# deadskull7/One-Stop-for-COVID-19-Infection-and-Lung-Segmentation-plus-Classification

Measured on AMD Instinct MI355X. Metric: CT images/sec (fwd+bwd) U-Net 512x512x1 bs16, higher is better.
Workload: dtype f32 storage / accumulate / parameters; conv products as a two-term fp16 split (3 fp16 MFMAs per multiply, ~2^-22 per product; --algo 2 = strict fp32); 1 GPU; U-Net infection seg (task1 graph T1:853-916), 512x512x1, batch 16/GPU, fp32, fwd+loss+bwd+Keras-Adam; BASELINE.json configs[1]; storage=fp32, global_batch=16, parallelism=dp1, deterministic=False, bn_fold=2

## Files before the change

### include/unet_hip.h

```cpp
#ifndef UNET_HIP_H
#define UNET_HIP_H
#include <stddef.h>
#include <stdint.h>

#ifdef __cplusplus
extern "C" {
#endif

#define UNET_ABI_VERSION 16

typedef struct unet_ctx unet_ctx;
typedef struct unet_model unet_model;
typedef uint16_t unet_bf16;
enum { UNET_DTYPE_F32 = 0, UNET_DTYPE_BF16 = 1 };

enum { UNET_OK = 0, UNET_E_ARG = -1, UNET_E_HIP = -2, UNET_E_SHAPE = -3, UNET_E_STATE = -4, UNET_E_NODEV = -5 };

enum { UNET_ALGO_AUTO = 0, UNET_ALGO_NAIVE = 1, UNET_ALGO_MFMA = 2 };

int32_t unet_abi_version(void);
int32_t unet_ctx_create(int32_t device_id, unet_ctx** out);
void unet_ctx_destroy(unet_ctx* ctx);
const char* unet_last_error(const unet_ctx* ctx);
int32_t unet_ctx_set_profiling(unet_ctx* ctx, int32_t on);
enum { UNET_OPT_RELU_BITS = 1, UNET_OPT_BN_FOLD = 2, UNET_OPT_ENC_BN_FUSED = 3, UNET_OPT_BN_CONCAT_ANALYTIC = 4, UNET_OPT_BN_FUSE_STATS = 5, UNET_OPT_DETERMINISTIC = 6,
       UNET_OPT_HEAD_FUSED = 7, UNET_OPT_SKIP_RAW = 8, UNET_OPT_POOL_SUMS_FUSED = 9, UNET_OPT_HEAD_BWD_FUSED = 10, UNET_OPT_CONV_PP = 13 };
int32_t unet_ctx_set_option(unet_ctx* ctx, int32_t option, int32_t value);
int32_t unet_ctx_get_option(unet_ctx* ctx, int32_t option);

enum { UNET_ACT_NONE = 0, UNET_ACT_RELU = 1, UNET_ACT_ELU = 2 };
enum { UNET_MASK_NONE = 0, UNET_MASK_RELU = 1, UNET_MASK_ELU = 2, UNET_MASK_ELU_DROP = 3, UNET_MASK_RELU_BITS = 9  };

size_t unet_conv3x3_w_ws_floats(int32_t cin, int32_t cout);
int32_t unet_conv3x3_pick_algo(int32_t algo, int32_t wd, int32_t cin, int32_t cout);
double unet_conv3x3_exec_ratio(int32_t algo, int32_t h, int32_t wd, int32_t cin, int32_t cout);
double unet_conv3x3_wgrad_exec_ratio(int32_t algo, int32_t h, int32_t wd, int32_t cin, int32_t cout);
int32_t unet_request_bn_stats(unet_ctx*, int32_t c);
int32_t unet_relu_bits_supported(int32_t algo, int32_t h, int32_t wd, int32_t cin, int32_t cout);
size_t unet_relu_bits_bytes(int32_t n, int32_t h, int32_t wd, int32_t c);
int32_t unet_request_relu_bits(unet_ctx*, void* bits);
int32_t unet_allow_k_slices(unet_ctx*);
// ... 16 lines not shown
int32_t unet_conv3x3_bwd_weights(unet_ctx*, const float* x, const float* dy, float* dw, float* db,
                                 void* ws, size_t ws_bytes, int32_t n, int32_t h, int32_t wd,
                                 int32_t cin, int32_t cout, int32_t algo, void* stream);

int32_t unet_convT2x2_fwd(unet_ctx*, const float* x, const float* w, const float* bias, float* y,
                          int32_t ldy, int32_t n, int32_t h, int32_t wd, int32_t cin, int32_t cout,
                          int32_t algo, void* stream);
int32_t unet_convT2x2_bwd_data(unet_ctx*, const float* dy, int32_t lddy, const float* w,
                               const float* relu_src, float* dx, int32_t n, int32_t h, int32_t wd,
                               int32_t cin, int32_t cout, int32_t algo, void* stream);
size_t unet_convT2x2_bwd_weights_ws_bytes(int32_t n, int32_t h, int32_t wd, int32_t cin, int32_t cout);
int32_t unet_convT2x2_bwd_weights(unet_ctx*, const float* x, const float* dy, int32_t lddy,
                                  float* dw, float* db, void* ws, size_t ws_bytes, int32_t n,
                                  int32_t h, int32_t wd, int32_t cin, int32_t cout, int32_t algo,
                                  void* stream);

int32_t unet_bn_stats(unet_ctx*, const float* x, int32_t ldx, double* sums, int64_t pixels,
                      int32_t c, void* stream);
int32_t unet_bn_stats_concat(unet_ctx*, const float* x_up, int32_t ldx, const double* src_sums, double src_count, const float* src_gamma,
                             const float* src_beta, double* sums, int64_t pixels, int32_t c_up, int32_t c_skip, void* stream);
int32_t unet_bn_finalize_train(unet_ctx*, const double* sums, double count, const float* gamma,
                               const float* beta, float* moving_mean, float* moving_var,
                               float* bnp, int32_t c, void* stream);
int32_t unet_bn_finalize_infer(unet_ctx*, const float* gamma, const float* beta,
                               const float* moving_mean, const float* moving_var, float* bnp,
                               int32_t c, void* stream);
int32_t unet_bn_apply(unet_ctx*, const float* x, int32_t ldx, const float* bnp, float* y,
                      int32_t ldy, int64_t pixels, int32_t c, void* stream);
int32_t unet_bn_bwd_stats(unet_ctx*, const float* dy, int32_t lddy, const float* x, int32_t ldx,
                          const float* bnp, double* sums, int64_t pixels, int32_t c, void* stream);
// ... 248 lines not shown
```

### one-stop-for-covid-19-infection-and-lung-segmentation-plus-classification_amd/_lib.py

```python
from __future__ import annotations

import ctypes as C
import os

_HERE = os.path.dirname(os.path.abspath(__file__))
LIB_PATH = os.environ.get("COVIDSEG_AMD_LIB") or os.path.join(_HERE, "libunet_hip.so")
ABI_VERSION = 16
COMM_HANDLE_BYTES, COMM_MAX_WORLD, COMM_MAX_DOUBLES = 64, 8, 2048

ALGO_AUTO, ALGO_NAIVE, ALGO_MFMA = 0, 1, 2
OPTIONS = {"relu_bits": 1, "bn_fold": 2, "enc_bn_fused": 3, "bn_concat_analytic": 4, "bn_fuse_stats": 5, "deterministic": 6, "head_fused": 7, "skip_raw": 8, "pool_sums_fused": 9, "head_bwd_fused": 10, "conv_pp": 13}
ARCH_UNET, ARCH_UNETPP, ARCH_CLASSIFIER = 0, 1, 2
LOSSES = {"bce_dice_loss": 0, "binary_crossentropy": 1, "dice_loss": 2, "tversky_loss": 3, "weighted_bce_dice_loss": 4}
DTYPE_F32, DTYPE_BF16 = 0, 1
ACT_NONE, ACT_RELU, ACT_ELU = 0, 1, 2
MASK_NONE, MASK_RELU, MASK_ELU, MASK_ELU_DROP = 0, 1, 2, 3
PROG_FWD_TRAIN, PROG_BWD, PROG_FWD_INFER = 0, 1, 2
SYNC_BN_FWD, SYNC_LOSS, SYNC_BN_BWD, SYNC_GRAD_BUCKET = 0, 1, 2, 3

f32p = C.POINTER(C.c_float)
f64p = C.POINTER(C.c_double)
vp = C.c_void_p
i32, i64, u64, f32, f64, sz = C.c_int32, C.c_int64, C.c_uint64, C.c_float, C.c_double, C.c_size_t


class SyncPoint(C.Structure):
# ... 14 lines not shown
    "unet_conv3x3_wgrad_exec_ratio": (f64, [i32, i32, i32, i32, i32]),
    "unet_request_bn_stats": (i32, [vp, i32]),
    "unet_relu_bits_supported": (i32, [i32, i32, i32, i32, i32]),
    "unet_relu_bits_bytes": (sz, [i32, i32, i32, i32]),
    "unet_request_relu_bits": (i32, [vp, vp]),
    "unet_allow_k_slices": (i32, [vp]),
    "unet_ctx_max_kernel_scratch_bytes": (i32, [vp]),
    "unet_conv3x3_fwd": (i32, [vp, vp, vp, vp, vp, i32, i32, i32, i32, i32, i32, f32, u64, i32, vp, vp]),
    "unet_conv3x3_bwd_data": (i32, [vp, vp, vp, vp, i32, f32, u64, vp, vp, i32, i32, i32, i32, i32, i32, vp]),
    "unet_conv3x3_bwd_weights_ws_bytes": (sz, [i32, i32, i32, i32, i32]),
    "unet_conv3x3_bwd_weights": (i32, [vp, vp, vp, vp, vp, vp, sz, i32, i32, i32, i32, i32, i32, vp]),
    "unet_convT2x2_fwd": (i32, [vp, vp, vp, vp, vp, i32, i32, i32, i32, i32, i32, i32, vp]),
    "unet_convT2x2_bwd_data": (i32, [vp, vp, i32, vp, vp, vp, i32, i32, i32, i32, i32, i32, vp]),
    "unet_convT2x2_bwd_weights_ws_bytes": (sz, [i32, i32, i32, i32, i32]),
    "unet_convT2x2_bwd_weights": (i32, [vp, vp, vp, i32, vp, vp, vp, sz, i32, i32, i32, i32, i32, i32, vp]),
    "unet_cast_f32_to_bf16": (i32, [vp, vp, vp, i64, vp]),
    "unet_cast_bf16_to_f32": (i32, [vp, vp, vp, i64, vp]),
    "unet_conv3x3_fwd_bf16": (i32, [vp, vp, vp, vp, vp, i32, i32, i32, i32, i32, i32, f32, u64, vp, vp]),
    "unet_conv3x3_first_fwd_bf16": (i32, [vp, vp, vp, vp, vp, i32, i32, i32, i32, i32, f32, u64, vp]),
    "unet_conv3x3_bwd_data_bf16": (i32, [vp, vp, vp, vp, i32, f32, u64, vp, vp, i32, i32, i32, i32, i32, vp]),
    "unet_conv3x3_bwd_weights_ws_bytes_bf16": (sz, [i32, i32, i32, i32, i32]),
    "unet_conv3x3_bwd_weights_bf16": (i32, [vp, vp, vp, vp, vp, vp, sz, i32, i32, i32, i32, i32, vp]),
    "unet_conv3x3_first_bwd_weights_bf16": (i32, [vp, vp, vp, vp, vp, vp, sz, i32, i32, i32, i32, vp]),
    "unet_convT2x2_fwd_bf16": (i32, [vp, vp, vp, vp, vp, i32, i32, i32, i32, i32, i32, vp, vp]),
    "unet_convT2x2_bwd_data_bf16": (i32, [vp, vp, i32, vp, vp, vp, i32, i32, i32, i32, i32, vp, vp]),
    "unet_convT2x2_bwd_weights_ws_bytes_bf16": (sz, [i32, i32, i32, i32, i32]),
    "unet_convT2x2_bwd_weights_bf16": (i32, [vp, vp, vp, i32, vp, vp, vp, sz, i32, i32, i32, i32, i32, vp]),
    "unet_bn_stats": (i32, [vp, vp, i32, vp, i64, i32, vp]),
    "unet_bn_stats_bf16": (i32, [vp, vp, i32, vp, i64, i32, vp]),
    "unet_conv3x3_bnfold_supported": (i32, [i32, i32, i32, i32, i32]),
# ... 198 lines not shown
```

### one-stop-for-covid-19-infection-and-lung-segmentation-plus-classification_amd/csrc/common.h

```cpp
#pragma once
#include <hip/hip_runtime.h>
#include <stdint.h>
#include <stdio.h>
#include <set>
#include <string>

#include "../../include/unet_hip.h"

constexpr int UNET_BN_SLOTS = 64, UNET_BN_SLOTS_DET = 1024, UNET_BN_SLOT_DOUBLES = 2048;
struct unet_loss_sel { int32_t kind = UNET_LOSS_BCE_DICE; float alpha = 0.5f, beta = 0.5f; };
inline bool unet_loss_sel_ok(const unet_loss_sel& ls, const float* wm = nullptr, bool need_map = true) {
  if (ls.kind < UNET_LOSS_BCE_DICE || ls.kind > UNET_LOSS_WEIGHTED_BCE_DICE) return false;
  if (ls.kind == UNET_LOSS_TVERSKY && !(ls.alpha > 0.0f && ls.beta > 0.0f && ls.alpha < 1e30f && ls.beta < 1e30f)) return false;
  return !need_map || (ls.kind == UNET_LOSS_WEIGHTED_BCE_DICE) == (wm != nullptr);
}
constexpr int UNET_HEAD_SUMS = 100;
struct unet_ctx {
  int device = 0;
  int num_cu = 256;
  int profiling = 0;
  int opt_relu_bits = 1;
  int opt_bn_fold = 2;
  int opt_enc_bn_fused = 1;
  int opt_bn_concat_analytic = 1;
  int opt_bn_fuse_stats = 1;
  int opt_pool_sums_fused = 1;
  int opt_skip_raw = 1;
  int opt_head_fused = 1;
  int opt_head_bwd_fused = 1;
  int opt_conv_pp = 1;
  int opt_deterministic = 0;
  double* bn_slots = nullptr;
  int bn_nslots() const { return opt_deterministic ? UNET_BN_SLOTS_DET : UNET_BN_SLOTS; }
  void* convt_img = nullptr;
  size_t convt_img_bytes = 0;
  int k_slices_ok = 0;
  void* splitk_ws = nullptr;
  size_t splitk_ws_bytes = 0;
  int stats_req_c = 0;
  const void* stats_in_slots = nullptr;
  int stats_in_slots_c = 0;
  bool stats_in_slots_xs = false;
  unsigned long long* signs_req = nullptr;
  const void* signs_done = nullptr;
  std::set<const void*> big_lds_kernels;
// ... 270 lines not shown
int32_t k_convT_naive_dgrad(unet_ctx*, const float* dy, int lddy, const float* w, const float* mask, float* dx,
                            int n, int h, int wd, int cin, int cout, hipStream_t s);
int32_t k_convT_naive_wgrad(unet_ctx*, const float* x, const float* dy, int lddy, float* dw, float* db, int n,
                            int h, int wd, int cin, int cout, hipStream_t s);
bool mfma_conv3x3_supported(int cin, int cout);
int32_t k_conv3x3_mfma_fwd(unet_ctx*, const float* x, const float* w, const float* bias, const float* mask, int mask_mode,
                           float* y, int n, int h, int wd, int cin, int cout, int act, float rate, uint64_t seed, hipStream_t s);
bool mfma_wgrad_supported(int ca, int cb);
bool mfma_convT_supported(int cin, int cout);
int32_t k_convT_mfma_fwd(unet_ctx*, const float* x, const float* w, const float* bias, float* y, int ldy, int n, int h, int wd,
                         int cin, int cout, hipStream_t s);
int32_t k_convT_mfma_dgrad(unet_ctx*, const float* dy, int lddy, const float* w, const float* mask, float* dx, int n, int h, int wd,
                           int cin, int cout, hipStream_t s);
size_t mfma_convT_wgrad_ws_bytes(int n, int h, int wd, int cin, int cout);
bool h2_convT_wgrad_selected(int algo, int cin, int cout);
size_t h2_convT_wgrad_ws_bytes(int n, int h, int wd, int cin, int cout);
int32_t k_convT_h2_wgrad(unet_ctx*, const float* x, const float* dy, int lddy, float* dw, float* db, void* ws, size_t ws_bytes, int n, int h, int wd, int cin, int cout,
                         hipStream_t s);
int32_t k_convT_mfma_wgrad(unet_ctx*, const float* x, const float* dy, int lddy, float* dw, float* db, void* ws, size_t ws_bytes, int n,
                           int h, int wd, int cin, int cout, hipStream_t s);
size_t mfma_wgrad_ws_bytes(int n, int h, int wd, int cin, int cout);
int32_t k_conv3x3_mfma_wgrad(unet_ctx*, const float* x, const float* dy, float* dw, float* db, void* ws,
                             size_t ws_bytes, int n, int h, int wd, int cin, int cout, hipStream_t s);
bool bf16_conv3x3_supported(int cin, int cout);
bool bf16_convT_supported(int cin, int cout);
bool bf16_wgrad_supported(int ca, int cb);
int32_t k_conv3x3_bf16_fwd(unet_ctx*, const unet_bf16* x, const float* w, const float* bias, const unet_bf16* mask, int mask_mode, unet_bf16* y, int n, int h,
                           int wd, int cin, int cout, int act, float rate, uint64_t seed, unet_bf16* wimg, int flip, hipStream_t s,
                           const unet_bf16* prepared = nullptr);
struct unet_wimg_prep { const float* w; unet_bf16* img; long long tap_stride, sk, sm, total8; int nb, nchunks, flip, m; };
// ... 19 lines not shown
```

### one-stop-for-covid-19-infection-and-lung-segmentation-plus-classification_amd/csrc/kernels_wgrad_h2.hip

```cpp
#include <stdlib.h>

#include <algorithm>

#include "common.h"

namespace {

typedef _Float16 f16x8 __attribute__((ext_vector_type(8)));
typedef _Float16 f16x2 __attribute__((ext_vector_type(2)));
typedef short s16x4 __attribute__((ext_vector_type(4)));
typedef short s16x8 __attribute__((ext_vector_type(8)));
typedef unet_f32x16 f32x16;

__device__ __forceinline__ void split2(float a, float b, unsigned& h, unsigned& m) {
  const f16x2 hh = __builtin_convertvector((unet_f32x2){a, b}, f16x2);
  const f16x2 mm = __builtin_convertvector((unet_f32x2){a - (float)hh[0], b - (float)hh[1]}, f16x2);
  h = __builtin_bit_cast(unsigned, hh); m = __builtin_bit_cast(unsigned, mm);
}
__device__ __forceinline__ float pow2f(int e) { return __uint_as_float((unsigned)(e + 127) << 23); }

__device__ __forceinline__ f16x8 lds_tr_frag(const char* p0, const char* p1) {
  typedef __attribute__((address_space(3))) s16x4 lds_s16x4;
  const s16x4 a = __builtin_amdgcn_ds_read_tr16_b64_v4i16((lds_s16x4*)(p0));
  const s16x4 b = __builtin_amdgcn_ds_read_tr16_b64_v4i16((lds_s16x4*)(p1));
// ... 518 lines not shown
  const long long pairs = (long long)p.tiles_a * p.tiles_b, per = 4LL * ca * cb;
  const long long units = (long long)n * p.strips;
  long long want = std::max<long long>(1, 512 / pairs);
  want = std::min(want, std::max<long long>(1, (64LL << 20) / per));
  p.units = (int)units; p.upb = (int)std::max<long long>(1, units / want);
  const long long ublocks = (units + p.upb - 1) / p.upb;
  long long cps = std::max<long long>(1, want / ublocks);
  cps = std::min<long long>(cps, std::max<long long>(1, h / 4));
  int rpc = (int)((h + cps - 1) / cps); rpc = (rpc + p.R - 1) / p.R * p.R;
  p.rows_per_chunk = rpc; p.chunks_per_strip = (h + rpc - 1) / rpc;
  p.nsplit = (int)(ublocks * p.chunks_per_strip); p.nslabs = p.nsplit;
  p.floats = (size_t)p.nslabs * (per + ca) + wgrad_reduce_scratch_floats(4, ca, cb, ca, p.nslabs);
  return p;
}

struct WgPlanH2 { int WA, WB, WR, tiles_a, tiles_b, strips, rows_per_chunk, chunks_per_strip, nsplit, nslabs, units, upb; size_t floats; };

constexpr int wgrad_h2_rows() { return 2; }

WgPlanH2 plan_wgrad_h2(int n, int h, int w, int ca, int cb) {
  WgPlanH2 p;
  int R = wgrad_h2_rows();
  p.WA = (ca % 64) == 0 ? 2 : 1; p.WB = (cb % 64) == 0 ? 2 : 1;
  p.WR = 4 / (p.WA * p.WB);
  if (p.WR > R) R = 4;
  p.tiles_a = (ca + 32 * p.WA - 1) / (32 * p.WA); p.tiles_b = (cb + 32 * p.WB - 1) / (32 * p.WB); p.strips = (w + 31) / 32;
  const long long pairs = (long long)p.tiles_a * p.tiles_b, per = 9LL * ca * cb;
  const long long units = (long long)n * p.strips;
  const long long target = R == 4 && p.WA * p.WB > 1 ? 256LL : 512LL;
  long long want = std::max<long long>(1, target / pairs);
// ... 99 lines not shown
  const WgPlanT p = plan_wgradT_h2(n, h, wd, cout, cin);
  if (!ws || ws_bytes < p.floats * sizeof(float)) UNET_FAIL(ctx, UNET_E_ARG, "convT wgrad h2: workspace %zu < %zu bytes", ws_bytes, p.floats * sizeof(float));
  float* part = static_cast<float*>(ws);
  const long long S = 4LL * cout * cin + cout;
  const int npairs = p.tiles_a * p.tiles_b;
  const dim3 grid((unsigned)(8 * ((p.nsplit + 7) / 8) * npairs));
  if (p.WA == 2 && p.BW == 2) hipLaunchKernelGGL((wgradT_h2_kernel<2, 2, 1, 1, 2>), grid, dim3(256), 0, s, dy, lddy, x, part, n, h, wd, cout, cin, p.tiles_b, p.strips, p.rows_per_chunk, p.chunks_per_strip,
                                    p.nsplit, npairs, S, p.units, p.upb);
  else if (p.WA == 2) hipLaunchKernelGGL((wgradT_h2_kernel<2, 2, 1, 1>), grid, dim3(256), 0, s, dy, lddy, x, part, n, h, wd, cout, cin, p.tiles_b, p.strips, p.rows_per_chunk, p.chunks_per_strip,
                                    p.nsplit, npairs, S, p.units, p.upb);
  else hipLaunchKernelGGL((wgradT_h2_kernel<1, 2, 2, 2>), grid, dim3(256), 0, s, dy, lddy, x, part, n, h, wd, cout, cin, p.tiles_b, p.strips, p.rows_per_chunk, p.chunks_per_strip, p.nsplit,
                          npairs, S, p.units, p.upb);
  UNET_CHECK_LAUNCH(ctx, "wgradT_h2");
  return k_wgrad_reduce(ctx, part, p.nslabs, 4, cout, cin, cout, dw, db, s);
}
```

### one-stop-for-covid-19-infection-and-lung-segmentation-plus-classification_amd/csrc/model.hip

```cpp
#include <algorithm>
#include <functional>
#include <map>
#include <set>
#include <string>
#include <vector>

#include "common.h"

extern "C" {

int32_t unet_abi_version(void) { return UNET_ABI_VERSION; }

int32_t unet_ctx_create(int32_t device_id, unet_ctx** out) {
  if (!out) return UNET_E_ARG;
  *out = nullptr;
  int ndev = 0;
  if (hipGetDeviceCount(&ndev) != hipSuccess || ndev <= 0 || device_id < 0 || device_id >= ndev) return UNET_E_NODEV;
  hipDeviceProp_t prop;
  if (hipGetDeviceProperties(&prop, device_id) != hipSuccess) return UNET_E_NODEV;
  if (std::string(prop.gcnArchName).rfind("gfx950", 0) != 0) return UNET_E_NODEV;
  unet_ctx* c = new unet_ctx();
  c->device = device_id;
  c->num_cu = prop.multiProcessorCount;
  const size_t sb = sizeof(double) * UNET_BN_SLOTS_DET * UNET_BN_SLOT_DOUBLES;
// ... 20 lines not shown
int32_t unet_ctx_set_profiling(unet_ctx* ctx, int32_t on) { if (!ctx) return UNET_E_ARG; ctx->profiling = on; return UNET_OK; }

static int* ctx_option(unet_ctx* ctx, int32_t option) {
  switch (option) {
    case UNET_OPT_RELU_BITS: return &ctx->opt_relu_bits;
    case UNET_OPT_BN_FOLD: return &ctx->opt_bn_fold;
    case UNET_OPT_ENC_BN_FUSED: return &ctx->opt_enc_bn_fused;
    case UNET_OPT_BN_CONCAT_ANALYTIC: return &ctx->opt_bn_concat_analytic;
    case UNET_OPT_BN_FUSE_STATS: return &ctx->opt_bn_fuse_stats;
    case UNET_OPT_DETERMINISTIC: return &ctx->opt_deterministic;
    case UNET_OPT_HEAD_FUSED: return &ctx->opt_head_fused;
    case UNET_OPT_SKIP_RAW: return &ctx->opt_skip_raw;
    case UNET_OPT_POOL_SUMS_FUSED: return &ctx->opt_pool_sums_fused;
    case UNET_OPT_HEAD_BWD_FUSED: return &ctx->opt_head_bwd_fused;
    case UNET_OPT_CONV_PP: return &ctx->opt_conv_pp;
    default: return nullptr;
  }
}
int32_t unet_ctx_set_option(unet_ctx* ctx, int32_t option, int32_t value) {
  if (!ctx) return UNET_E_ARG;
  int* p = ctx_option(ctx, option);
  const int hi = option == UNET_OPT_BN_FOLD ? 3 : option == UNET_OPT_CONV_PP ? 2 : 1;
  if (!p || value < 0 || value > hi) UNET_FAIL(ctx, UNET_E_ARG, "ctx_set_option: option %d value %d", option, value);
  *p = value;
  return UNET_OK;
}
int32_t unet_ctx_get_option(unet_ctx* ctx, int32_t option) {
  if (!ctx) return UNET_E_ARG;
  const int* p = ctx_option(ctx, option);
  if (!p) UNET_FAIL(ctx, UNET_E_ARG, "ctx_get_option: unknown option %d", option);
// ... 287 lines not shown
}
size_t unet_conv3x3_bwd_weights_ws_bytes_bf16(int32_t n, int32_t h, int32_t wd, int32_t cin, int32_t cout) {
  if (cin == 1) return c1_wgrad_ws_bytes(cout);
  return bf16_wgrad_ws_bytes(n, h, wd, cin, cout);
}
int32_t unet_conv3x3_bwd_weights_bf16(unet_ctx* ctx, const unet_bf16* x, const unet_bf16* dy, float* dw, float* db, void* ws, size_t ws_bytes, int32_t n,
                                      int32_t h, int32_t wd, int32_t cin, int32_t cout, void* stream) {
  if (!ctx || !x || !dy || !dw || !db || n < 1 || h < 1 || wd < 1) UNET_FAIL(ctx, UNET_E_ARG, "conv3x3_bwd_weights_bf16: bad args");
  return k_conv3x3_bf16_wgrad(ctx, x, dy, dw, db, ws, ws_bytes, n, h, wd, cin, cout, as_stream(stream));
}
int32_t unet_conv3x3_first_bwd_weights_bf16(unet_ctx* ctx, const float* x, const unet_bf16* dy, float* dw, float* db, void* ws, size_t ws_bytes, int32_t n,
                                            int32_t h, int32_t wd, int32_t cout, void* stream) {
  if (!ctx || !x || !dy || !dw || !db || n < 1 || h < 1 || wd < 1) UNET_FAIL(ctx, UNET_E_ARG, "conv3x3_first_bwd_weights_bf16: bad args");
  return k_conv3x3_c1_wgrad_bf16(ctx, x, dy, dw, db, ws, ws_bytes, n, h, wd, cout, as_stream(stream));
}
int32_t unet_convT2x2_fwd_bf16(unet_ctx* ctx, const unet_bf16* x, const float* w, const float* bias, unet_bf16* y, int32_t ldy, int32_t n, int32_t h,
                               int32_t wd, int32_t cin, int32_t cout, void* w_ws, void* stream) {
  if (!ctx || !x || !w || !y || !w_ws || ldy < cout || (ldy & 7) || n < 1 || h < 1 || wd < 1) UNET_FAIL(ctx, UNET_E_ARG, "convT_fwd_bf16: bad args");
  return k_convT_bf16_fwd(ctx, x, w, bias, y, ldy, n, h, wd, cin, cout, static_cast<unet_bf16*>(w_ws), as_stream(stream));
}
int32_t unet_convT2x2_bwd_data_bf16(unet_ctx* ctx, const unet_bf16* dy, int32_t lddy, const float* w, const unet_bf16* relu_src, unet_bf16* dx, int32_t n,
                                    int32_t h, int32_t wd, int32_t cin, int32_t cout, void* w_ws, void* stream) {
  if (!ctx || !dy || !w || !dx || !w_ws || lddy < cout || (lddy & 7)) UNET_FAIL(ctx, UNET_E_ARG, "convT_bwd_data_bf16: bad args");
  return k_convT_bf16_dgrad(ctx, dy, lddy, w, relu_src, dx, n, h, wd, cin, cout, static_cast<unet_bf16*>(w_ws), as_stream(stream));
}
size_t unet_convT2x2_bwd_weights_ws_bytes_bf16(int32_t n, int32_t h, int32_t wd, int32_t cin, int32_t cout) { return bf16_convT_wgrad_ws_bytes(n, h, wd, cin, cout); }
int32_t unet_convT2x2_bwd_weights_bf16(unet_ctx* ctx, const unet_bf16* x, const unet_bf16* dy, int32_t lddy, float* dw, float* db, void* ws, size_t ws_bytes,
                                       int32_t n, int32_t h, int32_t wd, int32_t cin, int32_t cout, void* stream) {
  if (!ctx || !x || !dy || !dw || !db || lddy < cout || (lddy & 7)) UNET_FAIL(ctx, UNET_E_ARG, "convT_bwd_weights_bf16: bad args");
  return k_convT_bf16_wgrad(ctx, x, dy, lddy, dw, db, ws, ws_bytes, n, h, wd, cin, cout, as_stream(stream));
// ... 256 lines not shown
    int s = m->H, t = m->W, idx = 0;
    for (auto& l : m->layers) {
      (void)idx;
      if (l.kind != 0) continue;
      int lvl;
      if (l.name == "c5a" || l.name == "c5b") lvl = 4;
      else { int k = l.name[1] - '0'; lvl = (k <= 4) ? k - 1 : 9 - k; }
      int hs = s >> lvl, ts = t >> lvl;
      wgb = std::max(wgb, m->dt ? unet_conv3x3_bwd_weights_ws_bytes_bf16(m->N, hs, ts, l.cin, l.cout) : unet_conv3x3_bwd_weights_ws_bytes(m->N, hs, ts, l.cin, l.cout));
    }
    for (auto& l : m->layers) {
      if (l.kind != 1) continue;
      int k = l.name[1] - '0';
      int lvl = 10 - k;
      wgb = std::max(wgb, m->dt ? bf16_convT_wgrad_ws_bytes(m->N, s >> lvl, t >> lvl, l.cin, l.cout) : unet_convT2x2_bwd_weights_ws_bytes(m->N, s >> lvl, t >> lvl, l.cin, l.cout));
    }
  }
  m->wgrad_ws_bytes = wgb;
  m->off_wgrad_ws = cv.take((wgb + 3) / 4);
  m->ws_floats_train = cv.cur;
}

double nel(const Buf& b) { return (double)b.n * b.h * b.w * b.c; }

#define ADD_OP(vec, nm, fl, by, ...)                          \
  do {                                                        \
    Op _o; _o.name = (nm); _o.flops = (fl); _o.bytes = (by);  \
    _o.run = [=](hipStream_t s) -> int32_t __VA_ARGS__;       \
    (vec).push_back(std::move(_o));                           \
  } while (0)
// ... 408 lines not shown
      const TInfo a = m->tinfo.at(first), b = m->tinfo.at(last_tensor);
      SY.push_back({(int)BW.size() - 1, 3, false, (size_t)a.off * 4, b.off + b.count - a.off});
    };
    bool enc_split = false;
    const int dec[4] = {256, 128, 64, 32};
    for (int k = 9; k >= 6; --k) {
      int c = dec[k - 6]; std::string ks = std::to_string(k);
      std::string prev = (k == 6) ? "c5b" : "c" + std::to_string(k - 1) + "b";
      int cprev = (k == 6) ? 512 : dec[k - 7];
      conv_bwd("c" + ks + "b", "c" + ks + "a", c, c, true, true, "", m->fold_c_off.count("c" + ks + "a") != 0);
      conv_bwd("c" + ks + "a", "bn" + ks, 2 * c, c, true, false, m->fold_off.count("c" + ks + "a") ? "cat" + ks : "");
      flush_def();
      if (!m->fold_c_off.count("c" + ks + "a")) bn_bwd("bn" + ks, "bn" + ks, "cat" + ks, "cat" + ks, 2 * c, 0, m->fold_off.count("c" + ks + "a") != 0);
      const Buf ib = m->act.at(prev), ug = m->grad.at("u" + ks);
      const std::string un = "u" + ks;
      ADD_OP(BW, "convT_wgrad:" + un, 2.0 * 4 * cprev * c * nel(ib) / ib.c, eb * (nel(ib) + nel(ug)), {
        if (dt) return k_convT_bf16_wgrad(ctx, CBF(m->Av(prev)), CBF(m->Dv(un)), ug.ld, m->G(un + "/kernel"), m->G(un + "/bias"), m->wsf(m->off_wgrad_ws), m->wgrad_ws_bytes, ib.n, ib.h,
                                          ib.w, cprev, c, s);
        return unet_convT2x2_bwd_weights(ctx, m->A(prev), m->D(un), ug.ld, m->G(un + "/kernel"), m->G(un + "/bias"), m->wsf(m->off_wgrad_ws), m->wgrad_ws_bytes,
                                         ib.n, ib.h, ib.w, cprev, c, algo, s);
      });
      ADD_OP(BW, "convT_dgrad:" + un, 2.0 * 4 * cprev * c * nel(ib) / ib.c, eb * (2 * nel(ib) + nel(ug)), {
        if (dt) return k_convT_bf16_dgrad(ctx, CBF(m->Dv(un)), ug.ld, m->P(un + "/kernel"), CBF(m->Av(prev)), WBF(m->Dv(prev)), ib.n, ib.h, ib.w, cprev, c, WBF(static_cast<void*>(m->wsf(m->off_wt))), s);
        const auto so = m->sign_off.find(prev);
        const auto pb = m->wprep_b.find(un);
        const void* img = pb == m->wprep_b.end() ? nullptr : m->wsf(pb->second);
        if (so != m->sign_off.end()) return k_convT_h2_dgrad(ctx, m->D(un), ug.ld, m->P(un + "/kernel"), m->wsf(so->second), m->D(prev), ib.n, ib.h, ib.w, cprev, c, s, 1, img);
        if (img) return k_convT_h2_dgrad(ctx, m->D(un), ug.ld, m->P(un + "/kernel"), m->A(prev), m->D(prev), ib.n, ib.h, ib.w, cprev, c, s, 0, img);
        return unet_convT2x2_bwd_data(ctx, m->D(un), ug.ld, m->P(un + "/kernel"), m->A(prev), m->D(prev), ib.n, ib.h, ib.w, cprev, c, algo, s);
      });
      if (k == 7) bucket("u7/kernel", "out/bias");
      if (k == 6) bucket("u6/kernel", "c6b/bias");
    }
    conv_bwd("c5b", "c5a", 512, 512, true, true);
    conv_bwd("c5a", "p4", 256, 512, true, false, "", ctx->opt_enc_bn_fused != 0);
    if (!ctx->opt_enc_bn_fused) bucket("c5a/kernel", "c5b/bias");
    for (int k = 4; k >= 1; --k) {
      int c = ENC[k - 1]; std::string ks = std::to_string(k);
      const Buf xb = m->act.at("bn" + ks), gb = m->grad.at("bn" + ks);
      const std::string bnn = "bn" + ks, pn = "p" + ks;
      const size_t so = m->bn_bsum_off.at(bnn);
      if (ctx->opt_enc_bn_fused) {
        const std::string dn = "bn" + std::to_string(10 - k), cb = "c" + ks + "b";
        const size_t sod = m->bn_bsum_off.at(dn), bod = m->bnp_off.at(dn), bo = m->bnp_off.at(bnn);
        const Buf cbuf = m->act.at(cb), cg = m->grad.at(cb);
// ... 1001 lines not shown
```

Measured before the change: 1065 images/sec.

## Fuse convT 2x2 weight-grad and data-grad into one MFMA kernel for 64->32 layer

```diff
diff --git a/include/unet_hip.h b/include/unet_hip.h
--- a/include/unet_hip.h
+++ b/include/unet_hip.h
@@ -24,7 +24,7 @@
 const char* unet_last_error(const unet_ctx* ctx);
 int32_t unet_ctx_set_profiling(unet_ctx* ctx, int32_t on);
 enum { UNET_OPT_RELU_BITS = 1, UNET_OPT_BN_FOLD = 2, UNET_OPT_ENC_BN_FUSED = 3, UNET_OPT_BN_CONCAT_ANALYTIC = 4, UNET_OPT_BN_FUSE_STATS = 5, UNET_OPT_DETERMINISTIC = 6,
-       UNET_OPT_HEAD_FUSED = 7, UNET_OPT_SKIP_RAW = 8, UNET_OPT_POOL_SUMS_FUSED = 9, UNET_OPT_HEAD_BWD_FUSED = 10, UNET_OPT_CONV_PP = 13 };
+       UNET_OPT_HEAD_FUSED = 7, UNET_OPT_SKIP_RAW = 8, UNET_OPT_POOL_SUMS_FUSED = 9, UNET_OPT_HEAD_BWD_FUSED = 10, UNET_OPT_CONV_PP = 13, UNET_OPT_CONVT_BWD_FUSED = 14 };
 int32_t unet_ctx_set_option(unet_ctx* ctx, int32_t option, int32_t value);
 int32_t unet_ctx_get_option(unet_ctx* ctx, int32_t option);
 
@@ -71,6 +71,11 @@
                                   float* dw, float* db, void* ws, size_t ws_bytes, int32_t n,
                                   int32_t h, int32_t wd, int32_t cin, int32_t cout, int32_t algo,
                                   void* stream);
+int32_t unet_convT2x2_bwd_fused_supported(unet_ctx*, int32_t algo, int32_t cin, int32_t cout);
+size_t unet_convT2x2_bwd_fused_ws_bytes(int32_t n, int32_t h, int32_t wd, int32_t cin, int32_t cout);
+int32_t unet_convT2x2_bwd_fused(unet_ctx*, const float* x, const float* dy, int32_t lddy, const float* w, int32_t relu_mask, float* dx, int32_t accumulate,
+                                float* dw, float* db, void* ws, size_t ws_bytes, int32_t n, int32_t h, int32_t wd, int32_t cin, int32_t cout, int32_t algo,
+                                void* stream);
 
 int32_t unet_bn_stats(unet_ctx*, const float* x, int32_t ldx, double* sums, int64_t pixels,
                       int32_t c, void* stream);
diff --git a/one-stop-for-covid-19-infection-and-lung-segmentation-plus-classification_amd/_lib.py b/one-stop-for-covid-19-infection-and-lung-segmentation-plus-classification_amd/_lib.py
--- a/one-stop-for-covid-19-infection-and-lung-segmentation-plus-classification_amd/_lib.py
+++ b/one-stop-for-covid-19-infection-and-lung-segmentation-plus-classification_amd/_lib.py
@@ -9,7 +9,7 @@
 COMM_HANDLE_BYTES, COMM_MAX_WORLD, COMM_MAX_DOUBLES = 64, 8, 2048
 
 ALGO_AUTO, ALGO_NAIVE, ALGO_MFMA = 0, 1, 2
-OPTIONS = {"relu_bits": 1, "bn_fold": 2, "enc_bn_fused": 3, "bn_concat_analytic": 4, "bn_fuse_stats": 5, "deterministic": 6, "head_fused": 7, "skip_raw": 8, "pool_sums_fused": 9, "head_bwd_fused": 10, "conv_pp": 13}
+OPTIONS = {"relu_bits": 1, "bn_fold": 2, "enc_bn_fused": 3, "bn_concat_analytic": 4, "bn_fuse_stats": 5, "deterministic": 6, "head_fused": 7, "skip_raw": 8, "pool_sums_fused": 9, "head_bwd_fused": 10, "conv_pp": 13, "convt_bwd_fused": 14}
 ARCH_UNET, ARCH_UNETPP, ARCH_CLASSIFIER = 0, 1, 2
 LOSSES = {"bce_dice_loss": 0, "binary_crossentropy": 1, "dice_loss": 2, "tversky_loss": 3, "weighted_bce_dice_loss": 4}
 DTYPE_F32, DTYPE_BF16 = 0, 1
@@ -54,6 +54,9 @@
     "unet_convT2x2_bwd_data": (i32, [vp, vp, i32, vp, vp, vp, i32, i32, i32, i32, i32, i32, vp]),
     "unet_convT2x2_bwd_weights_ws_bytes": (sz, [i32, i32, i32, i32, i32]),
     "unet_convT2x2_bwd_weights": (i32, [vp, vp, vp, i32, vp, vp, vp, sz, i32, i32, i32, i32, i32, i32, vp]),
+    "unet_convT2x2_bwd_fused_supported": (i32, [vp, i32, i32, i32]),
+    "unet_convT2x2_bwd_fused_ws_bytes": (sz, [i32, i32, i32, i32, i32]),
+    "unet_convT2x2_bwd_fused": (i32, [vp, vp, vp, i32, vp, i32, vp, i32, vp, vp, vp, sz, i32, i32, i32, i32, i32, i32, vp]),
     "unet_cast_f32_to_bf16": (i32, [vp, vp, vp, i64, vp]),
     "unet_cast_bf16_to_f32": (i32, [vp, vp, vp, i64, vp]),
     "unet_conv3x3_fwd_bf16": (i32, [vp, vp, vp, vp, vp, i32, i32, i32, i32, i32, i32, f32, u64, vp, vp]),
diff --git a/one-stop-for-covid-19-infection-and-lung-segmentation-plus-classification_amd/csrc/common.h b/one-stop-for-covid-19-infection-and-lung-segmentation-plus-classification_amd/csrc/common.h
--- a/one-stop-for-covid-19-infection-and-lung-segmentation-plus-classification_amd/csrc/common.h
+++ b/one-stop-for-covid-19-infection-and-lung-segmentation-plus-classification_amd/csrc/common.h
@@ -29,6 +29,7 @@
   int opt_head_fused = 1;
   int opt_head_bwd_fused = 1;
   int opt_conv_pp = 1;
+  int opt_convt_bwd_fused = 1;
   int opt_deterministic = 0;
   double* bn_slots = nullptr;
   int bn_nslots() const { return opt_deterministic ? UNET_BN_SLOTS_DET : UNET_BN_SLOTS; }
@@ -329,6 +330,10 @@
                            int cin, int cout, hipStream_t s);
 size_t mfma_convT_wgrad_ws_bytes(int n, int h, int wd, int cin, int cout);
 bool h2_convT_wgrad_selected(int algo, int cin, int cout);
+bool h2_convT_bwd_fused_selected(const unet_ctx* ctx, int algo, int cin, int cout);
+size_t h2_convT_bwd_fused_ws_bytes(int n, int h, int wd, int cin, int cout);
+int32_t k_convT_h2_bwd_fused(unet_ctx*, const float* x, const float* dy, int lddy, const float* w, int relu_mask, float* dx, int accumulate, float* dw, float* db, void* ws,
+                             size_t ws_bytes, int n, int h, int wd, int cin, int cout, hipStream_t s, const void* prepared = nullptr);
 size_t h2_convT_wgrad_ws_bytes(int n, int h, int wd, int cin, int cout);
 int32_t k_convT_h2_wgrad(unet_ctx*, const float* x, const float* dy, int lddy, float* dw, float* db, void* ws, size_t ws_bytes, int n, int h, int wd, int cin, int cout,
                          hipStream_t s);
diff --git a/one-stop-for-covid-19-infection-and-lung-segmentation-plus-classification_amd/csrc/kernels_wgrad_h2.hip b/one-stop-for-covid-19-infection-and-lung-segmentation-plus-classification_amd/csrc/kernels_wgrad_h2.hip
--- a/one-stop-for-covid-19-infection-and-lung-segmentation-plus-classification_amd/csrc/kernels_wgrad_h2.hip
+++ b/one-stop-for-covid-19-infection-and-lung-segmentation-plus-classification_amd/csrc/kernels_wgrad_h2.hip
@@ -556,6 +556,263 @@
   return p;
 }
 
+constexpr int TB_PPL = 32 * 64 + 64, TB_ROWB = 2 * TB_PPL;
+constexpr int TB_A = 2 * TB_ROWB, TB_B = 2 * 32 * 64;
+constexpr int TB_STAGE1 = TB_A + TB_B;
+constexpr int TB_W = 16 * 64 * 32;
+constexpr int TB_PART = 4 * 32 * 128;
+constexpr int TB_SMEM = 2 * TB_STAGE1 + TB_W + TB_PART;
+__device__ __forceinline__ int tb_cell(int p, int c) { return p * 128 + ((c ^ (p & 7)) << 4); }
+
+__global__ __launch_bounds__(256, 2) void convT_bwd_h2_kernel(const float* __restrict__ A, int ldA, const float* __restrict__ B, const unet_bf16* __restrict__ wimg_hdr,
+                                                              float* __restrict__ dX, float* __restrict__ part, int N, int H, int W, int strips, int rows_per_chunk,
+                                                              int chunks_per_strip, int nsplit, long long pstride, int units, int upb, int relu_mask, int accumulate) {
+  constexpr int CA = 32, CB = 64, TAPS = 4;
+  extern __shared__ __attribute__((aligned(16))) char smem[];
+  __shared__ float s_bs[4][64];
+  __shared__ float s_amax[2][4];
+  char* const s_a = smem; char* const s_b = smem + TB_A;
+  char* const s_w = smem + 2 * TB_STAGE1; char* const s_part = s_w + TB_W;
+  const int tid = threadIdx.x, lane = tid & 63, l31 = lane & 31, hi = lane >> 5;
+  const int wave = __builtin_amdgcn_readfirstlane(tid >> 6);
+  const int kp = wave & 1, wb = wave >> 1;
+  const int split = blockIdx.x;
+  if (split >= nsplit) return;
+  const int chunk = split % chunks_per_strip; const int ublk = split / chunks_per_strip;
+  const int ya = chunk * rows_per_chunk;
+  const int yb = ya + rows_per_chunk < H ? ya + rows_per_chunk : H;
+  const int HA = 2 * H, WAI = 2 * W;
+
+  {
+    const uint4* src = reinterpret_cast<const uint4*>(wimg_hdr + 128);
+#pragma unroll
+    for (int k = 0; k < 8; ++k) *reinterpret_cast<uint4*>(s_w + (tid + k * 256) * 16) = src[tid + k * 256];
+  }
+  const float w_unscale = *reinterpret_cast<const float*>(wimg_hdr);
+
+  f32x16 acc[TAPS];
+#pragma unroll
+  for (int t = 0; t < TAPS; ++t)
+#pragma unroll
+    for (int r = 0; r < 16; ++r) acc[t][r] = 0.0f;
+  float bsum = 0.0f;
+  int e_a = 120, e_b = 120;
+
+  const int i16 = lane & 15, g4 = lane >> 4;
+  const int tr_px = kp * 16 + (g4 >> 1) * 8 + (i16 >> 2), tr_ch = ((g4 & 1) * 16 + (i16 & 3) * 4) * 2;
+  const int sw0 = ((g4 >> 1) * 2) & 3;
+  const int a_off0 = tr_px * 64 + ((((tr_ch >> 4) ^ sw0)) << 4) + (tr_ch & 15);
+  const int a_off1 = (tr_px + 4) * 64 + ((((tr_ch >> 4) ^ (sw0 + 1))) << 4) + (tr_ch & 15);
+  const int b_off0 = (wb * 32 + tr_px) * 64 + tr_ch, b_off1 = b_off0 + 4 * 64;
+  const int d_sw = (l31 >> 2) & 3;
+
+  const int q8 = tid & 7, pc = tid >> 3;
+  const int u1 = (ublk + 1) * upb < units ? (ublk + 1) * upb : units;
+  for (int unit = ublk * upb; unit < u1; ++unit) {
+    const int cs = unit % strips, n = unit / strips;
+    const int x0 = cs * 32;
+    const __amdgpu_buffer_rsrc_t rs_a = make_rsrc(A + (long long)n * HA * WAI * ldA, (long long)HA * WAI * ldA * 4);
+    const __amdgpu_buffer_rsrc_t rs_b = make_rsrc(B + (long long)n * H * W * CB, (long long)H * W * CB * 4);
+    int abase_t[2], bbase_t[2], aput[2];
+#pragma unroll
+    for (int half = 0; half < 2; ++half) {
+      const int gx = 2 * x0 + half * 32 + pc;
+      abase_t[half] = gx < WAI ? (gx * ldA + q8 * 4) * 4 : UNET_OOB;
+      const int j = half * 16 + (pc >> 1);
+      aput[half] = (pc & 1) * TB_PPL + j * 64 + ((((q8 >> 1) ^ ((j >> 2) & 3))) << 4) + (q8 & 1) * 8;
+    }
+#pragma unroll
+    for (int sub = 0; sub < 2; ++sub) bbase_t[sub] = x0 + pc < W ? ((x0 + pc) * CB + sub * 32 + q8 * 4) * 4 : UNET_OOB;
+    unet_u32x4 areg[4], breg[2];
+    auto issue_loads = [&](int ys) __attribute__((always_inline)) {
+#pragma unroll
+      for (int row = 0; row < 2; ++row)
+#pragma unroll
+        for (int half = 0; half < 2; ++half) areg[row * 2 + half] = __builtin_amdgcn_raw_buffer_load_b128(rs_a, abase_t[half], (2 * ys + row) * WAI * ldA * 4, 0);
+#pragma unroll
+      for (int sub = 0; sub < 2; ++sub) breg[sub] = __builtin_amdgcn_raw_buffer_load_b128(rs_b, bbase_t[sub], ys * W * CB * 4, 0);
+    };
+    auto post_amax = [&]() __attribute__((always_inline)) {
+      float ma = 0.f, mb = 0.f;
+#pragma unroll
+      for (int k = 0; k < 4; ++k)
+#pragma unroll
+        for (int j = 0; j < 4; ++j) ma = fmaxf(ma, fabsf(__uint_as_float(areg[k][j])));
+#pragma unroll
+      for (int k = 0; k < 2; ++k)
+#pragma unroll
+        for (int j = 0; j < 4; ++j) mb = fmaxf(mb, fabsf(__uint_as_float(breg[k][j])));
+      ma = wave_max_nonneg(ma); mb = wave_max_nonneg(mb);
+      if (lane == 0) { s_amax[0][wave] = ma; s_amax[1][wave] = mb; }
+    };
+    unsigned xsign = 0;
+    float un_x = 0.f;
+    auto store_lds = [&]() __attribute__((always_inline)) {
+      const float ma = fmaxf(fmaxf(s_amax[0][0], s_amax[0][1]), fmaxf(s_amax[0][2], s_amax[0][3]));
+      const float mb = fmaxf(fmaxf(s_amax[1][0], s_amax[1][1]), fmaxf(s_amax[1][2], s_amax[1][3]));
+      const int eba = __builtin_amdgcn_readfirstlane((int)((__float_as_uint(ma) >> 23) & 0xFF));
+      const int ebb = __builtin_amdgcn_readfirstlane((int)((__float_as_uint(mb) >> 23) & 0xFF));
+      int d = 0;
+      if (eba >= 11 && eba - 127 + e_a >= 15) {
+        const int da_ = 138 - eba - e_a;
+        bsum *= pow2f(max(da_, -126));
+        d += da_; e_a = 138 - eba;
+      }
+      if (ebb >= 11 && ebb - 127 + e_b >= 15) { d += 138 - ebb - e_b; e_b = 138 - ebb; }
+      if (d != 0) {
+        const float f = pow2f(max(d, -126));
+#pragma unroll
+        for (int t = 0; t < TAPS; ++t)
+#pragma unroll
+          for (int r = 0; r < 16; ++r) acc[t][r] *= f;
+      }
+      const float sa = pow2f(e_a), sb = pow2f(e_b);
+      un_x = pow2f(max(-e_a, -126)) * w_unscale;
+      auto put = [&](char* dst, const unet_u32x4& v, float sc) __attribute__((always_inline)) {
+        unsigned h0, m0, h1, m1;
+        split2_scaled(__uint_as_float(v[0]), __uint_as_float(v[1]), sc, h0, m0);
+        split2_scaled(__uint_as_float(v[2]), __uint_as_float(v[3]), sc, h1, m1);
+        *reinterpret_cast<uint2*>(dst) = make_uint2(h0, h1);
+        *reinterpret_cast<uint2*>(dst + TB_STAGE1) = make_uint2(m0, m1);
+      };
+#pragma unroll
+      for (int row = 0; row < 2; ++row)
+#pragma unroll
+        for (int half = 0; half < 2; ++half) put(s_a + row * TB_ROWB + aput[half], areg[row * 2 + half], sa);
+      xsign = 0;
+#pragma unroll
+      for (int sub = 0; sub < 2; ++sub) {
+        put(s_b + (sub * 32 + pc) * 64 + q8 * 8, breg[sub], sb);
+#pragma unroll
+        for (int j = 0; j < 4; ++j) xsign |= (__uint_as_float(breg[sub][j]) > 0.f ? 1u : 0u) << (sub * 4 + j);
+      }
+    };
+
+    issue_loads(ya);
+    post_amax();
+    __syncthreads();
+    store_lds();
+    __syncthreads();
+    for (int ys = ya; ys < yb; ++ys) {
+      const bool more = ys + 1 < yb;
+      if (more) issue_loads(ys + 1);
+      {
+        f16x8 ah[4], am[4];
+#pragma unroll
+        for (int ab = 0; ab < 4; ++ab) {
+          const char* ap = s_a + (ab >> 1) * TB_ROWB + (ab & 1) * TB_PPL;
+          ah[ab] = lds_tr_frag(ap + a_off0, ap + a_off1); am[ab] = lds_tr_frag(ap + TB_STAGE1 + a_off0, ap + TB_STAGE1 + a_off1);
+          if (wb == 0) {
+#pragma unroll
+            for (int j = 0; j < 8; ++j) bsum += (float)ah[ab][j] + (float)am[ab][j];
+          }
+        }
+        const f16x8 bh = lds_tr_frag(s_b + b_off0, s_b + b_off1), bm = lds_tr_frag(s_b + TB_STAGE1 + b_off0, s_b + TB_STAGE1 + b_off1);
+#pragma unroll
+        for (int ab = 0; ab < 4; ++ab) acc[ab] = __builtin_amdgcn_mfma_f32_32x32x16_f16(ah[ab], bm, acc[ab], 0, 0, 0);
+#pragma unroll
+        for (int ab = 0; ab < 4; ++ab) acc[ab] = __builtin_amdgcn_mfma_f32_32x32x16_f16(am[ab], bh, acc[ab], 0, 0, 0);
+#pragma unroll
+        for (int ab = 0; ab < 4; ++ab) acc[ab] = __builtin_amdgcn_mfma_f32_32x32x16_f16(ah[ab], bh, acc[ab], 0, 0, 0);
+      }
+      {
+        f32x16 dacc[2];
+#pragma unroll
+        for (int i = 0; i < 2; ++i)
+#pragma unroll
+          for (int r = 0; r < 16; ++r) dacc[i][r] = 0.0f;
+        f16x8 wf[4][2], px[4][2];
+#pragma unroll
+        for (int t = 0; t < 4; ++t)
+#pragma unroll
+          for (int p = 0; p < 2; ++p) {
+            const int kk = kp * 4 + t;
+            wf[t][p] = *reinterpret_cast<const f16x8*>(s_w + ((((kk * 2 + wb) * 2 + p) * 2 + hi) * 512 + l31 * 16));
+            px[t][p] = *reinterpret_cast<const f16x8*>(s_a + p * TB_STAGE1 + kp * TB_ROWB + (t >> 1) * TB_PPL + l31 * 64 + (((((t & 1) * 2 + hi) ^ d_sw)) << 4));
+          }
+#pragma unroll
+        for (int pr = 0; pr < 3; ++pr) {
+          constexpr int PW[3] = {0, 1, 0}, PX[3] = {1, 0, 0};
+#pragma unroll
+          for (int t = 0; t < 4; ++t) dacc[t & 1] = __builtin_amdgcn_mfma_f32_32x32x16_f16(wf[t][PW[pr]], px[t][PX[pr]], dacc[t & 1], 0, 0, 0);
+        }
+        char* const so = s_part + wave * (32 * 128);
+#pragma unroll
+        for (int q = 0; q < 4; ++q)
+          *reinterpret_cast<float4*>(so + tb_cell(l31, hi * 4 + q)) = make_float4(dacc[0][q * 4] + dacc[1][q * 4], dacc[0][q * 4 + 1] + dacc[1][q * 4 + 1],
+                                                                                   dacc[0][q * 4 + 2] + dacc[1][q * 4 + 2], dacc[0][q * 4 + 3] + dacc[1][q * 4 + 3]);
+      }
+      if (more) post_amax();
+      __syncthreads();
+      if (x0 + pc < W) {
+        float* const o = dX + (((long long)n * H + ys) * W + x0 + pc) * CB + q8 * 4;
+#pragma unroll
+        for (int sub = 0; sub < 2; ++sub) {
+          const float4 p0 = *reinterpret_cast<const float4*>(s_part + (sub * 2) * (32 * 128) + tb_cell(pc, q8));
+          const float4 p1 = *reinterpret_cast<const float4*>(s_part + (sub * 2 + 1) * (32 * 128) + tb_cell(pc, q8));
+          float v[4] = {(p0.x + p1.x) * un_x, (p0.y + p1.y) * un_x, (p0.z + p1.z) * un_x, (p0.w + p1.w) * un_x};
+          if (relu_mask) {
+#pragma unroll
+            for (int j = 0; j < 4; ++j) v[j] = ((xsign >> (sub * 4 + j)) & 1u) ? v[j] : 0.f;
+          }
+          float* const q = o + sub * 32;
+          if (accumulate) { const float4 old = *reinterpret_cast<const float4*>(q); v[0] += old.x; v[1] += old.y; v[2] += old.z; v[3] += old.w; }
+          __builtin_nontemporal_store(v[0], q); __builtin_nontemporal_store(v[1], q + 1); __builtin_nontemporal_store(v[2], q + 2); __builtin_nontemporal_store(v[3], q + 3);
+        }
+      }
+      if (more) store_lds();
+      __syncthreads();
+    }
+  }
+  const float un_a = pow2f(max(-e_a, -126));
+  const float un = un_a * pow2f(max(-e_b, -126));
+#pragma unroll
+  for (int t = 0; t < TAPS; ++t)
+#pragma unroll
+    for (int r = 0; r < 16; ++r) acc[t][r] *= un;
+  bsum *= un_a;
+  bsum += __shfl_xor(bsum, 32, 64);
+  float* const img = reinterpret_cast<float*>(smem) + (size_t)wb * (TAPS * 16 * 64);
+  s_bs[wave][lane] = bsum;
+  if (kp == 1) {
+#pragma unroll
+    for (int t = 0; t < TAPS; ++t)
+#pragma unroll
+      for (int r = 0; r < 16; ++r) img[(t * 16 + r) * 64 + lane] = acc[t][r];
+  }
+  __syncthreads();
+  if (kp != 0) return;
+#pragma unroll
+  for (int t = 0; t < TAPS; ++t)
+#pragma unroll
+    for (int r = 0; r < 16; ++r) acc[t][r] += img[(t * 16 + r) * 64 + lane];
+  bsum = s_bs[wave][lane] + s_bs[wave + 1][lane];
+  float* P = part + (long long)split * pstride;
+  const int bc = wb * 32 + l31;
+#pragma unroll
+  for (int t = 0; t < TAPS; ++t)
+#pragma unroll
+    for (int r = 0; r < 16; ++r) {
+      const int m = (r & 3) + 8 * (r >> 2) + 4 * hi;
+      P[((long long)t * CA + m) * CB + bc] = acc[t][r];
+    }
+  if (wb == 0 && lane < 32) P[(long long)TAPS * CA * CB + l31] = bsum;
+}
+
+struct TbPlan { int strips, rows_per_chunk, chunks_per_strip, nsplit, units, upb; size_t floats; };
+TbPlan plan_convT_bwd_h2(int n, int h, int w) {
+  TbPlan p;
+  p.strips = (w + 31) / 32;
+  const long long units = (long long)n * p.strips, want = 512;
+  p.units = (int)units; p.upb = (int)std::max<long long>(1, units / want);
+  const long long ublocks = (units + p.upb - 1) / p.upb;
+  long long cps = std::max<long long>(1, want / ublocks);
+  cps = std::min<long long>(cps, std::max<long long>(1, h / 4));
+  p.rows_per_chunk = (int)((h + cps - 1) / cps); p.chunks_per_strip = (h + p.rows_per_chunk - 1) / p.rows_per_chunk;
+  p.nsplit = (int)(ublocks * p.chunks_per_strip);
+  p.floats = (size_t)p.nsplit * (4 * 32 * 64 + 32) + wgrad_reduce_scratch_floats(4, 32, 64, 32, p.nsplit);
+  return p;
+}
 struct WgPlanH2 { int WA, WB, WR, tiles_a, tiles_b, strips, rows_per_chunk, chunks_per_strip, nsplit, nslabs, units, upb; size_t floats; };
 
 constexpr int wgrad_h2_rows() { return 2; }
@@ -685,3 +942,30 @@
   UNET_CHECK_LAUNCH(ctx, "wgradT_h2");
   return k_wgrad_reduce(ctx, part, p.nslabs, 4, cout, cin, cout, dw, db, s);
 }
+
+bool h2_convT_bwd_fused_selected(const unet_ctx* ctx, int algo, int cin, int cout) {
+  return ctx && ctx->opt_convt_bwd_fused && cin == 64 && cout == 32 && h2_convT_selected(ctx, algo, cin, cout) && h2_convT_wgrad_selected(algo, cin, cout);
+}
+size_t h2_convT_bwd_fused_ws_bytes(int n, int h, int wd, int cin, int cout) { return cin == 64 && cout == 32 ? plan_convT_bwd_h2(n, h, wd).floats * sizeof(float) : 0; }
+
+int32_t k_convT_h2_bwd_fused(unet_ctx* ctx, const float* x, const float* dy, int lddy, const float* w, int relu_mask, float* dx, int accumulate, float* dw, float* db, void* ws,
+                             size_t ws_bytes, int n, int h, int wd, int cin, int cout, hipStream_t s, const void* prepared) {
+  if (cin != 64 || cout != 32) UNET_FAIL(ctx, UNET_E_SHAPE, "convT bwd fused h2: cin=%d cout=%d unsupported (64 -> 32)", cin, cout);
+  if (4LL * h * wd * lddy * 4 >= (1LL << 30) || (long long)h * wd * cin * 4 >= (1LL << 30)) UNET_FAIL(ctx, UNET_E_SHAPE, "convT bwd fused h2: one image must stay below 1 GiB (32-bit buffer offsets)");
+  const TbPlan p = plan_convT_bwd_h2(n, h, wd);
+  if (!ws || ws_bytes < p.floats * sizeof(float)) UNET_FAIL(ctx, UNET_E_ARG, "convT bwd fused h2: workspace %zu < %zu bytes", ws_bytes, p.floats * sizeof(float));
+  if (!prepared) {
+    const float* wl[1] = {w}; void* is[1] = {ctx->convt_img}; const int kind = 3;
+    int32_t r = k_h2_prep_multi(ctx, wl, nullptr, is, &cin, &cout, &kind, 1, s);
+    if (r) return r;
+    prepared = ctx->convt_img;
+  }
+  float* part = static_cast<float*>(ws);
+  const long long S = 4LL * cout * cin + cout;
+  UNET_BIG_LDS(ctx, convT_bwd_h2_kernel, (size_t)TB_SMEM, "convT_bwd_h2");
+  unet_note_kernel(ctx, reinterpret_cast<const void*>(convT_bwd_h2_kernel));
+  hipLaunchKernelGGL(convT_bwd_h2_kernel, dim3((unsigned)p.nsplit), dim3(256), (size_t)TB_SMEM, s, dy, lddy, x, static_cast<const unet_bf16*>(prepared), dx, part, n, h, wd, p.strips,
+                     p.rows_per_chunk, p.chunks_per_strip, p.nsplit, S, p.units, p.upb, relu_mask, accumulate);
+  UNET_CHECK_LAUNCH(ctx, "convT_bwd_h2");
+  return k_wgrad_reduce(ctx, part, p.nsplit, 4, cout, cin, cout, dw, db, s);
+}
diff --git a/one-stop-for-covid-19-infection-and-lung-segmentation-plus-classification_amd/csrc/model.hip b/one-stop-for-covid-19-infection-and-lung-segmentation-plus-classification_amd/csrc/model.hip
--- a/one-stop-for-covid-19-infection-and-lung-segmentation-plus-classification_amd/csrc/model.hip
+++ b/one-stop-for-covid-19-infection-and-lung-segmentation-plus-classification_amd/csrc/model.hip
@@ -58,6 +58,7 @@
     case UNET_OPT_POOL_SUMS_FUSED: return &ctx->opt_pool_sums_fused;
     case UNET_OPT_HEAD_BWD_FUSED: return &ctx->opt_head_bwd_fused;
     case UNET_OPT_CONV_PP: return &ctx->opt_conv_pp;
+    case UNET_OPT_CONVT_BWD_FUSED: return &ctx->opt_convt_bwd_fused;
     default: return nullptr;
   }
 }
@@ -375,6 +376,21 @@
   if (!ctx || !x || !dy || !dw || !db || n < 1 || h < 1 || wd < 1) UNET_FAIL(ctx, UNET_E_ARG, "conv3x3_first_bwd_weights_bf16: bad args");
   return k_conv3x3_c1_wgrad_bf16(ctx, x, dy, dw, db, ws, ws_bytes, n, h, wd, cout, as_stream(stream));
 }
+int32_t unet_convT2x2_bwd_fused_supported(unet_ctx* ctx, int32_t algo, int32_t cin, int32_t cout) { return h2_convT_bwd_fused_selected(ctx, algo, cin, cout) ? 1 : 0; }
+size_t unet_convT2x2_bwd_fused_ws_bytes(int32_t n, int32_t h, int32_t wd, int32_t cin, int32_t cout) {
+  return std::max(unet_convT2x2_bwd_weights_ws_bytes(n, h, wd, cin, cout), h2_convT_bwd_fused_ws_bytes(n, h, wd, cin, cout));
+}
+int32_t unet_convT2x2_bwd_fused(unet_ctx* ctx, const float* x, const float* dy, int32_t lddy, const float* w, int32_t relu_mask, float* dx, int32_t accumulate, float* dw,
+                                float* db, void* ws, size_t ws_bytes, int32_t n, int32_t h, int32_t wd, int32_t cin, int32_t cout, int32_t algo, void* stream) {
+  if (!ctx || !x || !dy || !w || !dx || !dw || !db || lddy < cout || n < 1 || h < 1 || wd < 1) UNET_FAIL(ctx, UNET_E_ARG, "convT_bwd_fused: bad args");
+  if (h2_convT_bwd_fused_selected(ctx, algo, cin, cout) && ws && ws_bytes >= h2_convT_bwd_fused_ws_bytes(n, h, wd, cin, cout))
+    return k_convT_h2_bwd_fused(ctx, x, dy, lddy, w, relu_mask, dx, accumulate, dw, db, ws, ws_bytes, n, h, wd, cin, cout, as_stream(stream));
+  if (accumulate) UNET_FAIL(ctx, UNET_E_SHAPE, "convT_bwd_fused: accumulating into dx goes with the fused kernel (cin=%d cout=%d)", cin, cout);
+  int32_t r = unet_convT2x2_bwd_weights(ctx, x, dy, lddy, dw, db, ws, ws_bytes, n, h, wd, cin, cout, algo, stream);
+  if (r) return r;
+  return unet_convT2x2_bwd_data(ctx, dy, lddy, w, relu_mask ? x : nullptr, dx, n, h, wd, cin, cout, algo, stream);
+}
+
 int32_t unet_convT2x2_fwd_bf16(unet_ctx* ctx, const unet_bf16* x, const float* w, const float* bias, unet_bf16* y, int32_t ldy, int32_t n, int32_t h,
                                int32_t wd, int32_t cin, int32_t cout, void* w_ws, void* stream) {
   if (!ctx || !x || !w || !y || !w_ws || ldy < cout || (ldy & 7) || n < 1 || h < 1 || wd < 1) UNET_FAIL(ctx, UNET_E_ARG, "convT_fwd_bf16: bad args");
@@ -661,6 +677,7 @@
       int k = l.name[1] - '0';
       int lvl = 10 - k;
       wgb = std::max(wgb, m->dt ? bf16_convT_wgrad_ws_bytes(m->N, s >> lvl, t >> lvl, l.cin, l.cout) : unet_convT2x2_bwd_weights_ws_bytes(m->N, s >> lvl, t >> lvl, l.cin, l.cout));
+      if (!m->dt && h2_convT_bwd_fused_selected(m->ctx, m->algo, l.cin, l.cout)) wgb = std::max(wgb, h2_convT_bwd_fused_ws_bytes(m->N, s >> lvl, t >> lvl, l.cin, l.cout));
     }
   }
   m->wgrad_ws_bytes = wgb;
@@ -1099,6 +1116,14 @@
       if (!m->fold_c_off.count("c" + ks + "a")) bn_bwd("bn" + ks, "bn" + ks, "cat" + ks, "cat" + ks, 2 * c, 0, m->fold_off.count("c" + ks + "a") != 0);
       const Buf ib = m->act.at(prev), ug = m->grad.at("u" + ks);
       const std::string un = "u" + ks;
+      const auto pbf = m->wprep_b.find(un);
+      if (!dt && pbf != m->wprep_b.end() && h2_convT_bwd_fused_selected(ctx, algo, cprev, c)) {
+        const size_t imgo = pbf->second;
+        ADD_OP(BW, "convT_bwd:" + un, 2.0 * 2.0 * 4 * cprev * c * nel(ib) / ib.c, eb * (2 * nel(ib) + nel(ug)), {
+          return k_convT_h2_bwd_fused(ctx, m->A(prev), m->D(un), ug.ld, m->P(un + "/kernel"), 1, m->D(prev), 0, m->G(un + "/kernel"), m->G(un + "/bias"), m->wsf(m->off_wgrad_ws),
+                                      m->wgrad_ws_bytes, ib.n, ib.h, ib.w, cprev, c, s, m->wsf(imgo));
+        });
+      } else {
       ADD_OP(BW, "convT_wgrad:" + un, 2.0 * 4 * cprev * c * nel(ib) / ib.c, eb * (nel(ib) + nel(ug)), {
         if (dt) return k_convT_bf16_wgrad(ctx, CBF(m->Av(prev)), CBF(m->Dv(un)), ug.ld, m->G(un + "/kernel"), m->G(un + "/bias"), m->wsf(m->off_wgrad_ws), m->wgrad_ws_bytes, ib.n, ib.h,
                                           ib.w, cprev, c, s);
@@ -1114,6 +1139,7 @@
         if (img) return k_convT_h2_dgrad(ctx, m->D(un), ug.ld, m->P(un + "/kernel"), m->A(prev), m->D(prev), ib.n, ib.h, ib.w, cprev, c, s, 0, img);
         return unet_convT2x2_bwd_data(ctx, m->D(un), ug.ld, m->P(un + "/kernel"), m->A(prev), m->D(prev), ib.n, ib.h, ib.w, cprev, c, algo, s);
       });
+      }
       if (k == 7) bucket("u7/kernel", "out/bias");
       if (k == 6) bucket("u6/kernel", "c6b/bias");
     }
```

Result: no change. 1072 images/sec, median of 6 (+0.7%).
